# telegraphroad/VCNF

Hardware: AMD Instinct MI355X
Metric: flow transforms/sec (log_prob + sample), D=64 RQ-spline, batch=1M (higher is better)
Workload: dtype f32 results on fp16x3 split operands: every fp32 operand of a conditioner GEMM travels as hi + lo fp16 halves, three f16 matrix instructions per product (four in the 48- and 16-deep layers), fp32 accumulation; measured against fp64 (tests/test_gpu_gemm_error.py): GEMM error 0.6-0.75x the exact-fp32

## Files before the change

### vcnf_amd/csrc/fused_layer_v6.hip

```cpp
#include <hip/hip_runtime.h>
#include <stdint.h>

#include "../../include/vcnf_hip.h"
#include "rqs_math.hpp"
#include "fused_common.hpp"
#include "rqs_lean.hpp"
#include "split_half.hpp"

#ifndef VCNF_ABL
#define VCNF_ABL 0
#endif
#ifndef VCNF_TIME
#define VCNF_TIME 0
#endif
#ifndef VCNF_AHEAD
#define VCNF_AHEAD 1
#endif
#if VCNF_TIME
#define VCNF_T(I) { const long long t_ = clock64(); tacc[I] += t_ - tlast; tlast = t_; }
#define VCNF_TIME_PARAM , float* tstamps
#define VCNF_TIME_ARG , time_buffer()
#else
#define VCNF_T(I)
#define VCNF_TIME_PARAM
#define VCNF_TIME_ARG
#endif

#define VCNF_SYNC() { __builtin_amdgcn_sched_barrier(0); asm volatile("s_waitcnt lgkmcnt(0)\n\ts_barrier" ::: "memory"); __builtin_amdgcn_sched_barrier(0); }

namespace vcnf {

#if VCNF_TIME
constexpr int kTimeSlots = 24;
static float* time_buffer() {
  static float* buf = nullptr;
  if (!buf && hipMalloc(&buf, 2 * kTimeSlots * sizeof(float)) != hipSuccess) buf = nullptr;
  return buf;
}
extern "C" int vcnf_v6_phase_stamps(float* out) {
  if (!time_buffer() || hipDeviceSynchronize() != hipSuccess) return VCNF_ERR_LAUNCH;
  return hipMemcpy(out, time_buffer(), 2 * kTimeSlots * sizeof(float), hipMemcpyDeviceToHost) == hipSuccess ? VCNF_OK : VCNF_ERR_LAUNCH;
}
#endif

template <int DI, int DT, int C, int H, int NBLK, int K, bool INV>
__global__ __launch_bounds__(512, 2) void fused_rqs_layer_v6_kernel(const FusedArgs a VCNF_TIME_PARAM) {
  static_assert(H == 128 && K == 8, "4 row blocks of 32 over 4 waves; 3 K - 1 = 23 logits: two features per 48 rows");
  static_assert((DI == 16 || DI == 32) && DT == DI && (C == 0 || C == 16), "shape family");
  constexpr int kBlock = 512;
  constexpr int kTile = 128;
  constexpr int NCB = 4;
  constexpr int D = DI + DT;
  constexpr int XS = D + 4;
  constexpr int NTX = DI / 16;
  constexpr int NTC = C / 16;
  constexpr int NT0 = NTX + NTC;
  constexpr int NTH = H / 16;
  constexpr int P = 3 * K - 1;
  constexpr int NG = DT / 4;
  constexpr int NR = NG / 2;
  constexpr int TABW = 3 * (K + 1);
  using L = PackLayout6<DI, DT, C, H, NBLK, K>;
  constexpr int GFRAG = 3 * NTH * 2 * 64;
  constexpr int RING = VCNF_AHEAD + 1;

  extern __shared__ __align__(16) float smem[];
  uint4* act = reinterpret_cast<uint4*>(smem);
  uint4* act_hi = act;
  uint4* act_lo = act + NTH * NCB * 64;
  float* xt = smem + 2 * GFRAG * 4;
  uint4* ctxf = reinterpret_cast<uint4*>(xt + kTile * XS);
  float* tab = reinterpret_cast<float*>(ctxf + (C > 0 ? NCB * 2 * 64 : 0));
  float* ldt = tab + ((DI * TABW + 3) & ~3);
  int* tfi = reinterpret_cast<int*>(ldt + kTile);
  int* idi = tfi + DT;
  constexpr int NBV = C > 0 ? 3 : 2;
  constexpr int NBT = 1 + NBLK * NBV;
  constexpr int BPL = NG * 48 + NBT * (H / 2);
  float* biasf = reinterpret_cast<float*>(idi + DI + 4);
  float* ldold = biasf + 2 * BPL;
  int* tflag = reinterpret_cast<int*>(ldold + kTile);

  const int tid = threadIdx.x;
  const int lane = tid & 63;
  const int wave = __builtin_amdgcn_readfirstlane(tid >> 6);
  const int rp = wave & 3;
  const int ch = wave >> 2;
  const int c32 = lane & 31;
  const int kg = lane >> 5;
  const RqsConst& c = a.c;
  const bool shared = a.sh_w != nullptr;
  const LeanConst lc = make_lean_const(c);

  if (ch == 1) __builtin_amdgcn_s_setprio(1);
  for (int i = tid; i < NG * 96; i += kBlock) {
    const int g = i / 96, hf = i % 96 / 48;
    biasf[hf * BPL + g * 48 + i % 48] = a.wpack[L::BF + i];
  }
  for (int i = tid; i < NBT * H; i += kBlock) {
    const int v = i / H, blk = (v - 1) / NBV, sel = (v - 1) % NBV, r = i % H;
    const int off = v == 0 ? L::B0 : L::BLK0 + blk * L::BLK + (sel == 0 ? L::BA : sel == 1 ? L::BB : L::BC);
    biasf[(r >> 4 & 1) * BPL + NG * 48 + v * (H / 2) + (r >> 5) * 16 + (r & 15)] = a.wpack[off + r];
  }
  for (int i = tid; i < DT; i += kBlock) tfi[i] = a.tf_idx[i];
  for (int i = tid; i < DI; i += kBlock) idi[i] = a.id_idx[i];
  if (shared) {
    for (int i = tid; i < 3 * DI; i += kBlock) {
      const int f = i % DI;
      SplitLogits p{a.sh_w + f * K, a.sh_h + f * K, a.sh_d + f * (K - 1), K, 1.f, c.edge_logit, c.tails};
      rqs_build_table_part_k<K>(p, c, tab + f * TABW, 1, i / DI);
    }
  }

  const __amdgpu_buffer_rsrc_t wr =
      __builtin_amdgcn_make_buffer_rsrc(const_cast<float*>(a.wpack), 0, a.wpack_bytes, 0x00020000);
  const int voff = lane * 16;
  const float* bplane = biasf + kg * BPL;

  const long long ntiles = (a.B + kTile - 1) / kTile;
  bool bad = false;
  float satm = 0.f;
#if VCNF_TIME
  long long tacc[20], tlast = clock64();
  const long long tstart = tlast, rstart = wall_clock64();
  for (int i = 0; i < 20; ++i) tacc[i] = 0;
#endif
  float4 xpre[kTile * (D / 4) / kBlock], cpre[1];
  static_assert(kTile * (D / 4) % kBlock == 0 && (C == 0 || kTile * (C / 4) == kBlock), "rows per thread");
#define VCNF_PREFETCH_ROWS(TILE)                                                          \
  {                                                                                       \
    const long long pb0 = min((TILE) * kTile, a.B);                                       \
    const long long left = (a.B - pb0) * (D * 4);                                         \
    const __amdgpu_buffer_rsrc_t xr_ = __builtin_amdgcn_make_buffer_rsrc(                 \
        const_cast<float*>(a.x) + pb0 * D, 0, (int)min(left, (long long)(kTile * D * 4)), 0x00020000); \
    _Pragma("unroll") for (int k = 0; k < kTile * (D / 4) / kBlock; ++k)                  \
      xpre[k] = __builtin_bit_cast(float4, __builtin_amdgcn_raw_buffer_load_b128(xr_, (tid + kBlock * k) * 16, 0, 0)); \
    if (C > 0) {                                                                          \
      const long long leftc = (a.B - pb0) * (C * 4);                                      \
      const __amdgpu_buffer_rsrc_t cr_ = __builtin_amdgcn_make_buffer_rsrc(               \
          const_cast<float*>(a.ctx) + pb0 * C, 0, (int)min(leftc, (long long)(kTile * C * 4)), 0x00020000); \
      cpre[0] = __builtin_bit_cast(float4, __builtin_amdgcn_raw_buffer_load_b128(cr_, tid * 16, 0, 0)); \
    }                                                                                     \
  }
#define VCNF_ROWS_ARRIVED()                                                               \
  {                                                                                       \
    _Pragma("unroll") for (int k = 0; k < kTile * (D / 4) / kBlock; ++k) {                \
      floatx4 v_ = __builtin_bit_cast(floatx4, xpre[k]);                                  \
      asm volatile("" : "+v"(v_));                                                        \
      xpre[k] = __builtin_bit_cast(float4, v_);                                           \
    }                                                                                     \
    if (C > 0) {                                                                          \
      floatx4 v_ = __builtin_bit_cast(floatx4, cpre[0]);                                  \
      asm volatile("" : "+v"(v_));                                                        \
      cpre[0] = __builtin_bit_cast(float4, v_);                                           \
    }                                                                                     \
  }
  VCNF_PREFETCH_ROWS((long long)blockIdx.x)
  VCNF_ROWS_ARRIVED()
  for (long long tile = blockIdx.x; tile < ntiles; tile += gridDim.x) {
    const long long b0 = tile * kTile;
    const int rows = (int)min((long long)kTile, a.B - b0);
    satm = 0.f;
    { VCNF_T(0) VCNF_SYNC(); VCNF_T(15) }
    {
      constexpr int D4 = D / 4;
      if (tid == 0) *tflag = 0;
#pragma unroll
      for (int k = 0; k < kTile * D4 / kBlock; ++k) {
        const int i = tid + kBlock * k;
        const int r = i / D4, o = i - r * D4;
        *reinterpret_cast<float4*>(xt + r * XS + 4 * o) = xpre[k];
      }
      if (C > 0) {
        const int r = tid >> 2, part = tid & 3;
        half4 h4, l4;
        const float cv[4] = {cpre[0].x, cpre[0].y, cpre[0].z, cpre[0].w};
#pragma unroll
        for (int i = 0; i < 4; ++i) satm = fmaxf(satm, cv[i] == cv[i] ? __builtin_fabsf(cv[i]) : __builtin_inff());
        asm volatile("" : "+v"(satm));
#pragma unroll
        for (int i = 0; i < 4; ++i) {
          const float x = __builtin_amdgcn_fmed3f(cv[i], -65504.f, 65504.f);
          const _Float16 hv = (_Float16)x;
          h4[i] = hv;
          l4[i] = (_Float16)((x - (float)hv) * kLoScale);
        }
        const int at = (((r >> 5) * 2) * 64 + (r & 31) + 32 * (part >> 1));
        uint2* dh = reinterpret_cast<uint2*>(ctxf + at) + (part & 1);
        uint2* dl = reinterpret_cast<uint2*>(ctxf + at + 64) + (part & 1);
        *dh = __builtin_bit_cast(uint2, h4);
        *dl = __builtin_bit_cast(uint2, l4);
      }
    }
    { VCNF_T(1) VCNF_SYNC(); VCNF_T(15) }

    {
      constexpr int UNR = DI / 4;
      const int mi = tid >> 2, part = tid & 3;
      float lsum = 0.f;
      float xv[UNR], fv[UNR];
      float* px[UNR];
#pragma unroll
      for (int k = 0; k < UNR; ++k) {
        px[k] = xt + mi * XS + idi[part * UNR + k];
        xv[k] = *px[k];
        fv[k] = xv[k];
      }
      if (shared) {
        float yv[UNR], lad[UNR];
        bool in_[UNR];
#pragma unroll
        for (int k = 0; k < UNR; ++k) {
          in_[k] = (xv[k] >= c.lo_x) && (xv[k] <= c.hi_x);
          bool bad1 = false;
          rqs_point_table_inside<INV, K>(in_[k] ? xv[k] : c.lo_x, tab + (part * UNR + k) * TABW, yv[k], lad[k], bad1);
          bad = bad || (bad1 && in_[k]);
        }
#pragma unroll
        for (int k = 0; k < UNR; ++k) {
          const float o = in_[k] ? yv[k] : xv[k];
          *px[k] = o;
          if (INV) fv[k] = o;
          lsum += in_[k] ? lad[k] : 0.f;
        }
      }
      lsum += __shfl_xor(lsum, 1, 64);
      lsum += __shfl_xor(lsum, 2, 64);
      int tid_ = tid;
      asm volatile("" : "+v"(tid_));
      if (part == 0) ldt[tid_ >> 2] = lsum;
#pragma unroll
      for (int k = 0; k < UNR; ++k) satm = fmaxf(satm, fv[k] == fv[k] ? 0.f : __builtin_inff());
      const int k0 = part * UNR;
      const int t0 = k0 >> 4, kg0 = (k0 >> 3) & 1;
      const int at = (t0 * NCB + (mi >> 5)) * 64 + (mi & 31) + 32 * kg0;
      if (UNR == 8) {
        half8 h8, l8;
        float f8[8];
#pragma unroll
        for (int k = 0; k < 8; ++k) f8[k] = fv[k < UNR ? k : 0];
        split8<false>(f8, h8, l8, satm);
        act_hi[at] = __builtin_bit_cast(uint4, h8);
        act_lo[at] = __builtin_bit_cast(uint4, l8);
      } else {
        half4 h4, l4;
        satm = fmaxf(fmaxf(satm, __builtin_fabsf(fv[0])), __builtin_fabsf(fv[1]));
        satm = fmaxf(fmaxf(satm, __builtin_fabsf(fv[2 < UNR ? 2 : 0])), __builtin_fabsf(fv[3 < UNR ? 3 : 0]));
        asm volatile("" : "+v"(satm));
#pragma unroll
        for (int i = 0; i < 4; ++i) {
          const float x = __builtin_amdgcn_fmed3f(fv[i < UNR ? i : 0], -65504.f, 65504.f);
          const _Float16 hv = (_Float16)x;
          h4[i] = hv;
          l4[i] = (_Float16)((x - (float)hv) * kLoScale);
        }
        reinterpret_cast<uint2*>(act_hi + at)[(k0 >> 2) & 1] = __builtin_bit_cast(uint2, h4);
        reinterpret_cast<uint2*>(act_lo + at)[(k0 >> 2) & 1] = __builtin_bit_cast(uint2, l4);
      }
    }
    { VCNF_T(2) VCNF_SYNC(); VCNF_T(15) }
    if (ch == 1) { VCNF_T(14) VCNF_SYNC(); VCNF_T(16) }

    half8 ahi[NTH], alo[NTH];
    floatx16 abias;
#define VCNF_LOAD_BIAS16(DST, VEC)                                                        \
  _Pragma("unroll") for (int i_ = 0; i_ < 4; ++i_) {                                      \
    const floatx4 b4_ = *reinterpret_cast<const floatx4*>(bplane + NG * 48 + (VEC) * (H / 2) + 16 * rp + 4 * i_); \
    DST[4 * i_ + 0] = b4_[0]; DST[4 * i_ + 1] = b4_[1]; DST[4 * i_ + 2] = b4_[2]; DST[4 * i_ + 3] = b4_[3]; \
  }
#define VCNF_LOAD_HIDDEN(WOFF, BVEC)                                                      \
  {                                                                                       \
    _Pragma("unroll") for (int t = 0; t < NTH; ++t) {                                     \
      ahi[t] = __builtin_bit_cast(half8, wload(wr, voff, 4 * ((WOFF) + ((rp * NTH + t) * 2 + 0) * 256))); \
      alo[t] = __builtin_bit_cast(half8, wload(wr, voff, 4 * ((WOFF) + ((rp * NTH + t) * 2 + 1) * 256))); \
    }                                                                                     \
    VCNF_LOAD_BIAS16(abias, BVEC)                                                         \
  }

    floatx16 h[2];
    {
      half8 w0h[NT0], w0l[NT0];
      floatx16 bias0;
#pragma unroll
      for (int t = 0; t < NT0; ++t) {
        w0h[t] = __builtin_bit_cast(half8, wload(wr, voff, 4 * (L::W0 + ((rp * NT0 + t) * 2 + 0) * 256)));
        w0l[t] = __builtin_bit_cast(half8, wload(wr, voff, 4 * (L::W0 + ((rp * NT0 + t) * 2 + 1) * 256)));
      }
      VCNF_LOAD_BIAS16(bias0, 0)
#pragma unroll
      for (int j = 0; j < 2; ++j) {
        const int cb = 2 * ch + j;
        floatx16 mainv = bias0, corr = {}, corr2 = {};
#pragma unroll
        for (int t = 0; t < NT0; ++t) {
          const half8 bh = __builtin_bit_cast(half8, t < NTX ? act_hi[(t * NCB + cb) * 64 + lane] : ctxf[(cb * 2 + 0) * 64 + lane]);
          const half8 bl = __builtin_bit_cast(half8, t < NTX ? act_lo[(t * NCB + cb) * 64 + lane] : ctxf[(cb * 2 + 1) * 64 + lane]);
          mainv = mfma32h(w0h[t], bh, mainv);
          corr = mfma32h(w0h[t], bl, corr);
          corr = mfma32h(w0l[t], bh, corr);
          corr2 = mfma32h(w0l[t], bl, corr2);
        }
#pragma unroll
        for (int r = 0; r < 16; ++r) h[j][r] = fmaf(fmaf(corr2[r], kLoUnscale, corr[r]), kLoUnscale, mainv[r]);
      }
    }
    { VCNF_T(3) VCNF_SYNC(); VCNF_T(15) }
#define VCNF_PUBLISH(SRC, RELU)                                                           \
  _Pragma("unroll") for (int j = 0; j < 2; ++j) {                                         \
    _Pragma("unroll") for (int hh = 0; hh < 2; ++hh) {                                    \
      float v8_[8];                                                                       \
      _Pragma("unroll") for (int i = 0; i < 8; ++i) v8_[i] = SRC[j][8 * hh + i];          \
      half8 h8_, l8_;                                                                     \
      split8<RELU>(v8_, h8_, l8_, satm);                                                  \
      const int at = ((2 * rp + hh) * NCB + 2 * ch + j) * 64 + lane;                      \
      act_hi[at] = __builtin_bit_cast(uint4, h8_);                                        \
      act_lo[at] = __builtin_bit_cast(uint4, l8_);                                        \
    }                                                                                     \
  }
    VCNF_LOAD_HIDDEN(L::BLK0 + L::WA, 1)
    VCNF_PUBLISH(h, true)
    { VCNF_T(4) VCNF_SYNC(); VCNF_T(15) }

#define VCNF_READ_B(T)                                                                    \
  {                                                                                       \
    rh[(T) % RING] = __builtin_bit_cast(half8, act_hi[((((T) & 7)) * NCB + 2 * ch + ((T) >> 3)) * 64 + lane]); \
    rl[(T) % RING] = __builtin_bit_cast(half8, act_lo[((((T) & 7)) * NCB + 2 * ch + ((T) >> 3)) * 64 + lane]); \
  }
#define VCNF_HIDDEN_COMPUTE(OUT)                                                          \
  {                                                                                       \
    half8 rh[RING], rl[RING];                 \
    floatx16 corr;                                                                        \
    _Pragma("unroll") for (int st_ = 0; st_ < VCNF_AHEAD; ++st_) {                        \
      VCNF_READ_B(st_)                                                                    \
    }                                                                                     \
    _Pragma("unroll") for (int st_ = 0; st_ < 2 * NTH; ++st_) {                           \
      const int j = st_ >> 3, tk_ = st_ & 7;                                              \
      if (st_ + VCNF_AHEAD < 2 * NTH) {                                                   \
        VCNF_READ_B(st_ + VCNF_AHEAD)                                                     \
      }                                                                                   \
      if (tk_ == 0) {                                                                       \
        OUT[j] = abias;                                                                   \
        corr = floatx16{};                                                                \
      }                                                                                   \
      OUT[j] = mfma32h(ahi[tk_], rh[st_ % RING], OUT[j]);                                      \
      corr = mfma32h(ahi[tk_], rl[st_ % RING], corr);                                          \
      corr = mfma32h(alo[tk_], rh[st_ % RING], corr);                                          \
      if (tk_ == NTH - 1) {                                                                 \
        _Pragma("unroll") for (int r = 0; r < 16; ++r) OUT[j][r] = fmaf(corr[r], kLoUnscale, OUT[j][r]); \
      }                                                                                   \
    }                                                                                     \
    __builtin_amdgcn_sched_group_barrier(0x100, 2 * VCNF_AHEAD, 0);                       \
    _Pragma("unroll") for (int st_ = 0; st_ + VCNF_AHEAD < 2 * NTH; ++st_) {              \
      __builtin_amdgcn_sched_group_barrier(0x100, 2, 0);                                  \
      __builtin_amdgcn_sched_group_barrier(0x008, 3, 0);                                  \
    }                                                                                     \
    __builtin_amdgcn_sched_group_barrier(0x008, 3 * VCNF_AHEAD, 0);                       \
  }

#pragma unroll
    for (int blk = 0; blk < (VCNF_ABL == 5 ? 0 : NBLK); ++blk) {
      const int base = L::BLK0 + blk * L::BLK;
      floatx16 t[2];
      VCNF_HIDDEN_COMPUTE(t)
      { VCNF_T(5) VCNF_SYNC(); VCNF_T(15) }
      VCNF_LOAD_HIDDEN(base + L::WB, 2 + blk * NBV)
      half8 wch, wcl;
      floatx16 gate[2], gbias;
      if (C > 0) {
        wch = __builtin_bit_cast(half8, wload(wr, voff, 4 * (base + L::WC + (rp * 2 + 0) * 256)));
        wcl = __builtin_bit_cast(half8, wload(wr, voff, 4 * (base + L::WC + (rp * 2 + 1) * 256)));
        VCNF_LOAD_BIAS16(gbias, 3 + blk * NBV)
      }
      VCNF_PUBLISH(t, true)
      { VCNF_T(6) VCNF_SYNC(); VCNF_T(15) }
      VCNF_HIDDEN_COMPUTE(t)
      if (C > 0 && VCNF_ABL != 6) {
#pragma unroll
        for (int j = 0; j < 2; ++j) {
          const half8 bh = __builtin_bit_cast(half8, ctxf[((2 * ch + j) * 2 + 0) * 64 + lane]);
          const half8 bl = __builtin_bit_cast(half8, ctxf[((2 * ch + j) * 2 + 1) * 64 + lane]);
          floatx16 corr = {}, corr2 = {};
          gate[j] = mfma32h(wch, bh, gbias);
          corr = mfma32h(wch, bl, corr);
          corr = mfma32h(wcl, bh, corr);
          corr2 = mfma32h(wcl, bl, corr2);
#pragma unroll
          for (int r = 0; r < 16; ++r) gate[j][r] = fmaf(fmaf(corr2[r], kLoUnscale, corr[r]), kLoUnscale, gate[j][r]);
        }
      }
      { VCNF_T(5) VCNF_SYNC(); VCNF_T(15) }
      if (blk + 1 < NBLK) {
        VCNF_LOAD_HIDDEN(base + L::BLK + L::WA, 1 + (blk + 1) * NBV)
      }
      if (C > 0 && VCNF_ABL != 6) {
#pragma unroll
        for (int j = 0; j < 2; ++j) {
#pragma unroll
          for (int r = 0; r < 16; ++r) {
            const float sg = hw_rcp(1.f + hw_exp2(-gate[j][r]));
            h[j][r] = fmaf(t[j][r], sg, h[j][r]);
          }
        }
      } else {
#pragma unroll
        for (int j = 0; j < 2; ++j) h[j] += t[j];
      }
      if (blk + 1 < NBLK) {
        VCNF_PUBLISH(h, true)
      } else {
        VCNF_PUBLISH(h, false)
      }
      { VCNF_T(7) VCNF_SYNC(); VCNF_T(15) }
    }
    if (ch == 0) { VCNF_T(14) VCNF_SYNC(); VCNF_T(17) }
#undef VCNF_HIDDEN_COMPUTE
#undef VCNF_READ_B
#undef VCNF_LOAD_HIDDEN
#undef VCNF_PUBLISH

    half8 fhi[NTH], flo[NTH];
#pragma unroll
    for (int t = 0; t < NTH; ++t) {
      fhi[t] = __builtin_bit_cast(half8, act_hi[(t * NCB + rp) * 64 + lane]);
      flo[t] = __builtin_bit_cast(half8, act_lo[(t * NCB + rp) * 64 + lane]);
    }
    float ld_acc = 0.f;
    uint4* win = act + ch * GFRAG;
    const int gtid = tid & 255;
    constexpr int NSTG = GFRAG / 256;
    static_assert(GFRAG % 256 == 0, "whole fragments per thread");
#define VCNF_STAGE_DMA(G)                                                                 \
  _Pragma("unroll") for (int k = 0; k < NSTG; ++k)                                        \
    dma16_to_lds(wr, win + (gtid & ~63) + k * 256, gtid * 16, 4 * (L::WF + (G) * (4 * GFRAG) + k * 1024));
    floatx16 pa[3];
#define VCNF_LOAD_BIASF(G)                                                                \
  _Pragma("unroll") for (int b = 0; b < 3; ++b) {                                         \
    _Pragma("unroll") for (int i_ = 0; i_ < 4; ++i_) {                                    \
      const floatx4 b4_ = *reinterpret_cast<const floatx4*>(bplane + (G) * 48 + 16 * b + 4 * i_); \
      pa[b][4 * i_ + 0] = b4_[0]; pa[b][4 * i_ + 1] = b4_[1]; pa[b][4 * i_ + 2] = b4_[2]; pa[b][4 * i_ + 3] = b4_[3]; \
    }                                                                                     \
  }
    VCNF_LOAD_BIASF(ch)
    { VCNF_T(8) VCNF_SYNC(); VCNF_T(15) }
    VCNF_STAGE_DMA(ch)
    if (ch == 0 && rp < 2 && a.ld_mode) {
      const __amdgpu_buffer_rsrc_t or_ = __builtin_amdgcn_make_buffer_rsrc(a.logdet + b0, 0, rows * 4, 0x00020000);
      __builtin_amdgcn_raw_ptr_buffer_load_lds(or_, (__attribute__((address_space(3))) void*)(ldold + rp * 64), 4,
                                               lane * 4, rp * 256, 0, 0);
    }
    wait_vector_memory();
    { VCNF_T(9) VCNF_SYNC(); VCNF_T(15) }
    if (ch == 1) { VCNF_T(14) VCNF_SYNC(); VCNF_T(18) }
    for (int rnd = 0; rnd < (VCNF_ABL == 3 ? 0 : NR); ++rnd) {
      const int g = 2 * rnd + ch;
      float* px[2];
      float xin[2];
#pragma unroll
      for (int f2 = 0; f2 < 2; ++f2) {
        px[f2] = xt + (rp * 32 + c32) * XS + tfi[4 * g + 2 * kg + f2];
        xin[f2] = *px[f2];
      }
      {
        half8 wh[RING], wl[RING];
        floatx16 corr;
#define VCNF_READ_W(T)                                                                    \
  {                                                                                       \
    wh[(T) % RING] = __builtin_bit_cast(half8, win[((T) * 2 + 0) * 64 + lane]);           \
    wl[(T) % RING] = __builtin_bit_cast(half8, win[((T) * 2 + 1) * 64 + lane]);           \
  }
#pragma unroll
        for (int u = 0; u < VCNF_AHEAD; ++u) {
          VCNF_READ_W(u)
        }
#pragma unroll
        for (int u = 0; u < 3 * NTH; ++u) {
          const int b = u >> 3, t = u & 7;
          if (u + VCNF_AHEAD < 3 * NTH) {
            VCNF_READ_W(u + VCNF_AHEAD)
          }
          if (t == 0) corr = floatx16{};
          pa[b] = mfma32h(wh[u % RING], fhi[t], pa[b]);
          corr = mfma32h(wh[u % RING], flo[t], corr);
          corr = mfma32h(wl[u % RING], fhi[t], corr);
          if (t == NTH - 1) {
#pragma unroll
            for (int r = 0; r < 16; ++r) pa[b][r] = fmaf(corr[r], kLoUnscale, pa[b][r]);
          }
        }
        __builtin_amdgcn_sched_group_barrier(0x100, 2 * VCNF_AHEAD, 0);
#pragma unroll
        for (int u = 0; u + VCNF_AHEAD < 3 * NTH; ++u) {
          __builtin_amdgcn_sched_group_barrier(0x100, 2, 0);
          __builtin_amdgcn_sched_group_barrier(0x008, 3, 0);
        }
        __builtin_amdgcn_sched_group_barrier(0x008, 3 * VCNF_AHEAD, 0);
#undef VCNF_READ_W
      }
      { VCNF_T(10) VCNF_SYNC(); VCNF_T(15) }
      {
        const bool more = rnd + 1 < NR;
        if (!more) {
          VCNF_PREFETCH_ROWS(tile + gridDim.x)
        }
        if (more && VCNF_ABL != 2) {
          VCNF_STAGE_DMA(g + 2)
        }
        float yv[2], lad[2];
#pragma unroll
        for (int f2 = 0; f2 < 2; ++f2) {
          float lg[P];
#pragma unroll
          for (int tl = 0; tl < P; ++tl) lg[tl] = pa[(24 * f2 + tl) >> 4][(24 * f2 + tl) & 15];
          rqs_lean_eval<8, INV>(xin[f2], lg, lc, yv[f2], lad[f2], bad);
        }
        *px[0] = yv[0];
        *px[1] = yv[1];
        ld_acc += lad[0] + lad[1];
        if (more) {
          VCNF_LOAD_BIASF(g + 2)
        }
      }
      if (rnd + 1 < NR && VCNF_ABL != 2) wait_vector_memory();
      { VCNF_T(11) VCNF_SYNC(); VCNF_T(15) }
    }
    if (ch == 0) { VCNF_T(14) VCNF_SYNC(); VCNF_T(19) }
#undef VCNF_PREFETCH_ROWS
#undef VCNF_STAGE_DMA
#undef VCNF_LOAD_BIASF

    ld_acc += __shfl_xor(ld_acc, 32, 64);
    if (ch == 1 && kg == 0) ldt[rp * 32 + c32] += ld_acc;
    if (satm > 65504.f) *tflag = 1;
    { VCNF_T(12) VCNF_SYNC(); VCNF_T(15) }
    VCNF_ROWS_ARRIVED()
#undef VCNF_ROWS_ARRIVED
    int tid_ = tid;
    asm volatile("" : "+v"(tid_));
    const bool over = *tflag != 0;
    if (tid == 0 && over && a.sat) atomicAdd(a.sat, 1);
    if (a.redo) {
      if (tid_ < kTile / kFusedFlagRows) {
        const __amdgpu_buffer_rsrc_t rr = __builtin_amdgcn_make_buffer_rsrc(
            a.redo + tile * (kTile / kFusedFlagRows), 0, 4 * ((rows + kFusedFlagRows - 1) / kFusedFlagRows), 0x00020000);
        __builtin_amdgcn_raw_buffer_store_b32(over ? 1 : 0, rr, tid_ * 4, 0, 0);
      }
      if (over) continue;
    }
    if (ch == 0 && (tid_ & 32) == 0) {
      const int mrow = (tid_ >> 6) * 32 + (tid_ & 31);
      const __amdgpu_buffer_rsrc_t lr = __builtin_amdgcn_make_buffer_rsrc(a.logdet + b0, 0, rows * 4, 0x00020000);
      const float o = a.ld_sign * (ld_acc + ldt[mrow]);
      __builtin_amdgcn_raw_buffer_store_b32(__builtin_bit_cast(unsigned, a.ld_mode ? ldold[mrow] + o : o), lr, mrow * 4, 0, 0);
    }
    {
      constexpr int D4 = D / 4;
      const __amdgpu_buffer_rsrc_t yr = __builtin_amdgcn_make_buffer_rsrc(a.y + b0 * D, 0, rows * (D * 4), 0x00020000);
      floatx4 yv[kTile * D4 / kBlock];
#pragma unroll
      for (int k = 0; k < kTile * D4 / kBlock; ++k) {
        const int i = tid_ + kBlock * k;
        const int r = i / D4, o = i - r * D4;
        yv[k] = *reinterpret_cast<const floatx4*>(xt + r * XS + 4 * o);
      }
#pragma unroll
      for (int k = 0; k < kTile * D4 / kBlock; ++k)
        __builtin_amdgcn_raw_buffer_store_b128(__builtin_bit_cast(__attribute__((ext_vector_type(4))) unsigned, yv[k]), yr, (tid_ + kBlock * k) * 16, 0, 0);
    }
  }
#if VCNF_TIME
  VCNF_T(13)
  if (blockIdx.x == 0 && (tid & 255) == 0 && tstamps) {
    float* ts = tstamps + (tid >> 8) * kTimeSlots;
    for (int i = 0; i < 20; ++i) ts[i] = (float)tacc[i];
    ts[20] = (float)(clock64() - tstart);
    ts[21] = (float)(wall_clock64() - rstart);
    ts[22] = (float)((ntiles - blockIdx.x + gridDim.x - 1) / gridDim.x);
  }
#endif
  if (INV && a.bad && bad) atomicAdd(a.bad, 1);
}

template <int DI, int DT, int C, int H, int NBLK, int K>
static int launch_v6(const FusedArgs& a, int inverse, hipStream_t st) {
  constexpr int D = DI + DT;
  constexpr int TILE = 128;
  constexpr size_t WIN = (size_t)2 * 3 * (H / 16) * 2 * 64 * 16;
  constexpr int NBT = 1 + NBLK * (C > 0 ? 3 : 2);
  const size_t lds = ((size_t)TILE * (D + 4) + ((DI * 3 * (K + 1) + 3) & ~3) + 2 * TILE + D + 8 + (DT / 4) * 96 + NBT * H) * 4 +
                     (C > 0 ? 4 * 2 * 64 * 16 : 0) + WIN + 64;
  static bool attr_set[2] = {false, false};
  if (!attr_set[inverse ? 1 : 0]) {
    hipError_t e;
    if (inverse)
      e = hipFuncSetAttribute(reinterpret_cast<const void*>(&fused_rqs_layer_v6_kernel<DI, DT, C, H, NBLK, K, true>),
                              hipFuncAttributeMaxDynamicSharedMemorySize, (int)lds);
    else
      e = hipFuncSetAttribute(reinterpret_cast<const void*>(&fused_rqs_layer_v6_kernel<DI, DT, C, H, NBLK, K, false>),
                              hipFuncAttributeMaxDynamicSharedMemorySize, (int)lds);
    if (e != hipSuccess) return VCNF_ERR_LAUNCH;
    attr_set[inverse ? 1 : 0] = true;
  }
  const long long ntiles = (a.B + TILE - 1) / TILE;
  dim3 grid((unsigned)(ntiles < 256 ? ntiles : 256));
  if (inverse)
    hipLaunchKernelGGL((fused_rqs_layer_v6_kernel<DI, DT, C, H, NBLK, K, true>), grid, dim3(512), lds, st, a VCNF_TIME_ARG);
  else
    hipLaunchKernelGGL((fused_rqs_layer_v6_kernel<DI, DT, C, H, NBLK, K, false>), grid, dim3(512), lds, st, a VCNF_TIME_ARG);
  return hipGetLastError() == hipSuccess ? VCNF_OK : VCNF_ERR_LAUNCH;
}

template <int NBLK>
static int launch_v6_family(const FusedArgs& a, int d_id, int ctx_dim, int inverse, hipStream_t st) {
#ifdef VCNF_DEV_ONLY
  return launch_v6<32, 32, 16, 128, NBLK, 8>(a, inverse, st);
#else
  if (d_id == 32) {
    return ctx_dim == 16 ? launch_v6<32, 32, 16, 128, NBLK, 8>(a, inverse, st)
                         : launch_v6<32, 32, 0, 128, NBLK, 8>(a, inverse, st);
  }
  return ctx_dim == 16 ? launch_v6<16, 16, 16, 128, NBLK, 8>(a, inverse, st)
                       : launch_v6<16, 16, 0, 128, NBLK, 8>(a, inverse, st);
#endif
}

#ifndef VCNF_V6_NBLK
#define VCNF_V6_NBLK 2
#endif
#if VCNF_V6_NBLK == 1
int launch_fused_v6_b1(const FusedArgs& a, int d_id, int ctx_dim, int inverse, hipStream_t st) {
  return launch_v6_family<1>(a, d_id, ctx_dim, inverse, st);
}
#elif VCNF_V6_NBLK == 2
int launch_fused_v6_b2(const FusedArgs& a, int d_id, int ctx_dim, int inverse, hipStream_t st) {
  return launch_v6_family<2>(a, d_id, ctx_dim, inverse, st);
}
#else
int launch_fused_v6_b3(const FusedArgs& a, int d_id, int ctx_dim, int inverse, hipStream_t st) {
  return launch_v6_family<3>(a, d_id, ctx_dim, inverse, st);
}
#endif

}
```

Before: 73.86 million.

## Defer forward identity-spline evaluation into wave-idle barrier slots and hoist loads

In the forward direction with shared identity-spline parameters, the per-feature table spline on identity dimensions moves out of the front of the tile. It now runs in phases where one wave group would otherwise sit waiting at a barrier, split between the two channel groups, with partial log-dets kept in a new LDS scratch array. The first-layer weight fragment loads are hoisted before the identity phase, and the old-logdet LDS DMA is issued at tile start with inline asm that sets m0. The goal is to overlap spline ALU work with the imbalance between wave groups, at the cost of extra LDS, more register pressure, and fragile inline asm.

```diff
diff --git a/vcnf_amd/csrc/fused_layer_v6.hip b/vcnf_amd/csrc/fused_layer_v6.hip
--- a/vcnf_amd/csrc/fused_layer_v6.hip
+++ b/vcnf_amd/csrc/fused_layer_v6.hip
@@ -31,7 +31,8 @@
 namespace vcnf {
 
 #if VCNF_TIME
-constexpr int kTimeSlots = 24;
+constexpr int kPhaseSlots = 24;
+constexpr int kTimeSlots = 28;
 static float* time_buffer() {
   static float* buf = nullptr;
   if (!buf && hipMalloc(&buf, 2 * kTimeSlots * sizeof(float)) != hipSuccess) buf = nullptr;
@@ -79,7 +80,8 @@
   constexpr int BPL = NG * 48 + NBT * (H / 2);
   float* biasf = reinterpret_cast<float*>(idi + DI + 4);
   float* ldold = biasf + 2 * BPL;
-  int* tflag = reinterpret_cast<int*>(ldold + kTile);
+  float* lpart = ldold + kTile;
+  int* tflag = reinterpret_cast<int*>(lpart + kBlock / 2);
 
   const int tid = threadIdx.x;
   const int lane = tid & 63;
@@ -121,9 +123,9 @@
   bool bad = false;
   float satm = 0.f;
 #if VCNF_TIME
-  long long tacc[20], tlast = clock64();
+  long long tacc[kPhaseSlots], tlast = clock64();
   const long long tstart = tlast, rstart = wall_clock64();
-  for (int i = 0; i < 20; ++i) tacc[i] = 0;
+  for (int i = 0; i < kPhaseSlots; ++i) tacc[i] = 0;
 #endif
   float4 xpre[kTile * (D / 4) / kBlock], cpre[1];
   static_assert(kTile * (D / 4) % kBlock == 0 && (C == 0 || kTile * (C / 4) == kBlock), "rows per thread");
@@ -162,6 +164,18 @@
     const int rows = (int)min((long long)kTile, a.B - b0);
     satm = 0.f;
     { VCNF_T(0) VCNF_SYNC(); VCNF_T(15) }
+    if (ch == 0 && rp < 2 && a.ld_mode) {
+      int tid_ = tid;
+      asm volatile("" : "+v"(tid_));
+      const unsigned long long base_ = reinterpret_cast<unsigned long long>(a.logdet + b0);
+      const __attribute__((ext_vector_type(4))) unsigned or_ = {(unsigned)base_, (unsigned)(base_ >> 32) & 0xffffu,
+                                                                (unsigned)rows * 4u, 0x00020000u};
+      const unsigned dst_ = (unsigned)reinterpret_cast<unsigned long long>(ldold) + rp * 256;
+      unsigned keep_;
+      asm volatile("s_nop 4\n\ts_mov_b32 %0, m0\n\ts_mov_b32 m0, %3\n\ts_nop 0\n\t"
+                   "buffer_load_dword %1, %2, %4 offen lds\n\ts_mov_b32 m0, %0"
+                   : "=&s"(keep_) : "v"((tid_ & 63) * 4), "s"(or_), "s"(dst_), "s"(rp * 256) : "memory");
+    }
     {
       constexpr int D4 = D / 4;
       if (tid == 0) *tflag = 0;
@@ -193,7 +207,46 @@
       }
     }
     { VCNF_T(1) VCNF_SYNC(); VCNF_T(15) }
-
+    half8 w0h[NT0], w0l[NT0];
+#pragma unroll
+    for (int t = 0; t < NT0; ++t) {
+      w0h[t] = __builtin_bit_cast(half8, wload(wr, voff, 4 * (L::W0 + ((rp * NT0 + t) * 2 + 0) * 256)));
+      w0l[t] = __builtin_bit_cast(half8, wload(wr, voff, 4 * (L::W0 + ((rp * NT0 + t) * 2 + 1) * 256)));
+    }
+
+    constexpr bool kSplineLate = !INV;
+#define VCNF_IDENTITY_SPLINE(K0, K1, LSUM)                                                \
+  {                                                                                       \
+    constexpr int UNR_ = DI / 4;                                                          \
+    int tid_ = tid;                           \
+    asm volatile("" : "+v"(tid_));                                                        \
+    const int part_ = tid_ & 3;                                                           \
+    float* px_[UNR_];                                                                     \
+    float xv_[UNR_], yv_[UNR_], lad_[UNR_];                                               \
+    bool in_[UNR_];                                                                       \
+    _Pragma("unroll") for (int k = (K0); k < (K1); ++k) {                                 \
+      px_[k] = xt + (tid_ >> 2) * XS + idi[part_ * UNR_ + k];                             \
+      xv_[k] = *px_[k];                                                                   \
+    }                                                                                     \
+    _Pragma("unroll") for (int k = (K0); k < (K1); ++k) {                                 \
+      in_[k] = (xv_[k] >= c.lo_x) && (xv_[k] <= c.hi_x);                                  \
+      bool bad1 = false;                                                                  \
+      rqs_point_table_inside<INV, K>(in_[k] ? xv_[k] : c.lo_x, tab + (part_ * UNR_ + k) * TABW, yv_[k], lad_[k], bad1); \
+      bad = bad || (bad1 && in_[k]);                                                      \
+    }                                                                                     \
+    _Pragma("unroll") for (int k = (K0); k < (K1); ++k) {                                 \
+      *px_[k] = in_[k] ? yv_[k] : xv_[k];                                                 \
+      LSUM += in_[k] ? lad_[k] : 0.f;                                                     \
+    }                                                                                     \
+  }
+#define VCNF_IDENTITY_LOGDET(LSUM)                                                        \
+  {                                                                                       \
+    LSUM += __shfl_xor(LSUM, 1, 64);                                                      \
+    LSUM += __shfl_xor(LSUM, 2, 64);                                                      \
+    int tid_ = tid;                                                                       \
+    asm volatile("" : "+v"(tid_));                                                        \
+    if ((tid_ & 3) == 0) ldt[tid_ >> 2] = LSUM;                                           \
+  }
     {
       constexpr int UNR = DI / 4;
       const int mi = tid >> 2, part = tid & 3;
@@ -206,7 +259,7 @@
         xv[k] = *px[k];
         fv[k] = xv[k];
       }
-      if (shared) {
+      if (shared && !kSplineLate) {
         float yv[UNR], lad[UNR];
         bool in_[UNR];
 #pragma unroll
@@ -224,11 +277,7 @@
           lsum += in_[k] ? lad[k] : 0.f;
         }
       }
-      lsum += __shfl_xor(lsum, 1, 64);
-      lsum += __shfl_xor(lsum, 2, 64);
-      int tid_ = tid;
-      asm volatile("" : "+v"(tid_));
-      if (part == 0) ldt[tid_ >> 2] = lsum;
+      if (!(shared && kSplineLate)) VCNF_IDENTITY_LOGDET(lsum)
 #pragma unroll
       for (int k = 0; k < UNR; ++k) satm = fmaxf(satm, fv[k] == fv[k] ? 0.f : __builtin_inff());
       const int k0 = part * UNR;
@@ -279,13 +328,7 @@
 
     floatx16 h[2];
     {
-      half8 w0h[NT0], w0l[NT0];
       floatx16 bias0;
-#pragma unroll
-      for (int t = 0; t < NT0; ++t) {
-        w0h[t] = __builtin_bit_cast(half8, wload(wr, voff, 4 * (L::W0 + ((rp * NT0 + t) * 2 + 0) * 256)));
-        w0l[t] = __builtin_bit_cast(half8, wload(wr, voff, 4 * (L::W0 + ((rp * NT0 + t) * 2 + 1) * 256)));
-      }
       VCNF_LOAD_BIAS16(bias0, 0)
 #pragma unroll
       for (int j = 0; j < 2; ++j) {
@@ -412,7 +455,16 @@
       }
       { VCNF_T(7) VCNF_SYNC(); VCNF_T(15) }
     }
-    if (ch == 0) { VCNF_T(14) VCNF_SYNC(); VCNF_T(17) }
+    if (ch == 0) {
+      if (kSplineLate && shared) {
+        float lsum = 0.f;
+        VCNF_IDENTITY_SPLINE(0, DI / 8, lsum)
+        int tid_ = tid;
+        asm volatile("" : "+v"(tid_));
+        lpart[tid_] = lsum;
+      }
+      { VCNF_T(21) VCNF_SYNC(); VCNF_T(17) }
+    }
 #undef VCNF_HIDDEN_COMPUTE
 #undef VCNF_READ_B
 #undef VCNF_LOAD_HIDDEN
@@ -443,14 +495,16 @@
     VCNF_LOAD_BIASF(ch)
     { VCNF_T(8) VCNF_SYNC(); VCNF_T(15) }
     VCNF_STAGE_DMA(ch)
-    if (ch == 0 && rp < 2 && a.ld_mode) {
-      const __amdgpu_buffer_rsrc_t or_ = __builtin_amdgcn_make_buffer_rsrc(a.logdet + b0, 0, rows * 4, 0x00020000);
-      __builtin_amdgcn_raw_ptr_buffer_load_lds(or_, (__attribute__((address_space(3))) void*)(ldold + rp * 64), 4,
-                                               lane * 4, rp * 256, 0, 0);
-    }
     wait_vector_memory();
     { VCNF_T(9) VCNF_SYNC(); VCNF_T(15) }
-    if (ch == 1) { VCNF_T(14) VCNF_SYNC(); VCNF_T(18) }
+    if (ch == 1) {
+      if (kSplineLate && shared) {
+        float lsum = 0.f;
+        VCNF_IDENTITY_SPLINE(0, DI / 4, lsum)
+        VCNF_IDENTITY_LOGDET(lsum)
+      }
+      { VCNF_T(20) VCNF_SYNC(); VCNF_T(18) }
+    }
     for (int rnd = 0; rnd < (VCNF_ABL == 3 ? 0 : NR); ++rnd) {
       const int g = 2 * rnd + ch;
       float* px[2];
@@ -523,7 +577,18 @@
       if (rnd + 1 < NR && VCNF_ABL != 2) wait_vector_memory();
       { VCNF_T(11) VCNF_SYNC(); VCNF_T(15) }
     }
-    if (ch == 0) { VCNF_T(14) VCNF_SYNC(); VCNF_T(19) }
+    if (ch == 0) {
+      if (kSplineLate && shared) {
+        int tid_ = tid;
+        asm volatile("" : "+v"(tid_));
+        float lsum = lpart[tid_];
+        VCNF_IDENTITY_SPLINE(DI / 8, DI / 4, lsum)
+        VCNF_IDENTITY_LOGDET(lsum)
+      }
+      { VCNF_T(22) VCNF_SYNC(); VCNF_T(19) }
+    }
+#undef VCNF_IDENTITY_SPLINE
+#undef VCNF_IDENTITY_LOGDET
 #undef VCNF_PREFETCH_ROWS
 #undef VCNF_STAGE_DMA
 #undef VCNF_LOAD_BIASF
@@ -571,10 +636,10 @@
   VCNF_T(13)
   if (blockIdx.x == 0 && (tid & 255) == 0 && tstamps) {
     float* ts = tstamps + (tid >> 8) * kTimeSlots;
-    for (int i = 0; i < 20; ++i) ts[i] = (float)tacc[i];
-    ts[20] = (float)(clock64() - tstart);
-    ts[21] = (float)(wall_clock64() - rstart);
-    ts[22] = (float)((ntiles - blockIdx.x + gridDim.x - 1) / gridDim.x);
+    for (int i = 0; i < kPhaseSlots; ++i) ts[i] = (float)tacc[i];
+    ts[kPhaseSlots + 0] = (float)(clock64() - tstart);
+    ts[kPhaseSlots + 1] = (float)(wall_clock64() - rstart);
+    ts[kPhaseSlots + 2] = (float)((ntiles - blockIdx.x + gridDim.x - 1) / gridDim.x);
   }
 #endif
   if (INV && a.bad && bad) atomicAdd(a.bad, 1);
@@ -586,7 +651,7 @@
   constexpr int TILE = 128;
   constexpr size_t WIN = (size_t)2 * 3 * (H / 16) * 2 * 64 * 16;
   constexpr int NBT = 1 + NBLK * (C > 0 ? 3 : 2);
-  const size_t lds = ((size_t)TILE * (D + 4) + ((DI * 3 * (K + 1) + 3) & ~3) + 2 * TILE + D + 8 + (DT / 4) * 96 + NBT * H) * 4 +
+  const size_t lds = ((size_t)TILE * (D + 4) + ((DI * 3 * (K + 1) + 3) & ~3) + 2 * TILE + 256 + D + 8 + (DT / 4) * 96 + NBT * H) * 4 +
                      (C > 0 ? 4 * 2 * 64 * 16 : 0) + WIN + 64;
   static bool attr_set[2] = {false, false};
   if (!attr_set[inverse ? 1 : 0]) {
```

New measurement: 73.91 million, median of 2. About the same (+0.1%).
